# cartographer-project/cartographer

Measured on AMD Instinct MI355X. Metric: candidate poses scored/sec, higher is better.
Workload: dtype u8/int32; 1 GPU; C2: 2D FastCorrelativeScanMatcher MatchFullSubmap (branch and bound): 1000-point scan vs 1 400x400 submap(s) per GPU, depth 7, full-angle search, m...; submaps_per_gpu=1, rotations=2373, found=1

## Files before the change

### cartographer_amd/csrc/cmx_common.h

```cpp
#ifndef CMX_COMMON_H_
#define CMX_COMMON_H_

#include <hip/hip_runtime.h>

#include <cstdarg>
#include <cstdint>
#include <cstdio>
#include <cstring>
#include <functional>
#include <mutex>
#include <string>
#include <vector>

#include "../../include/cartographer_mi355x.h"

namespace cmx {

void SetLastError(const char* fmt, ...);
const char* LastError();

struct HipError {
  cmx_status status;
};

// ... 1 lines not shown
  do {                                                                             \
    hipError_t cmx_err__ = (expr);                                                 \
    if (cmx_err__ != hipSuccess) {                                                 \
      ::cmx::SetLastError("%s failed: %s (%s:%d)", #expr,                          \
                          hipGetErrorString(cmx_err__), __FILE__, __LINE__);       \
      throw ::cmx::HipError{cmx_err__ == hipErrorOutOfMemory ? CMX_OUT_OF_MEMORY   \
                                                             : CMX_DEVICE_ERROR};  \
    }                                                                              \
  } while (0)

#define CMX_REQUIRE(cond, ...)                       \
  do {                                               \
    if (!(cond)) {                                   \
      ::cmx::SetLastError(__VA_ARGS__);              \
      throw ::cmx::HipError{CMX_INVALID_ARGUMENT};   \
    }                                                \
  } while (0)

template <typename F>
cmx_status Guard(F&& body) {
  try {
    body();
    return CMX_OK;
  } catch (const HipError& e) {
    return e.status;
  } catch (const std::bad_alloc&) {
    SetLastError("host allocation failed");
    return CMX_OUT_OF_MEMORY;
  } catch (const std::exception& e) {
    SetLastError("exception: %s", e.what());
    return CMX_DEVICE_ERROR;
  }
}

#define CMX_DEBUG_OPTIONS(X)                                                                      \
  X(rt2d_legacy)                 \
  X(rt2d_tile)                                        \
  X(rt2d_groups)                                   \
  X(rt2d_target)                                    \
  X(rt2d_lds_kb)                                         \
  X(rt2d_no_image_cache)             \
  X(rt2d_parts)                                 \
  X(rt2d_host_par)         \
  X(rt2d_tables_serial)    \
  X(rt2d_first_part)       \
  X(rt2d_image_kernels)    \
  X(rt2d_no_lane)          \
  X(rt2d_parts_pool)       \
  X(rt2d_grid_share)       \
  X(rt2d_unfused)            \
  X(rt2d_no_bounds)        \
  X(rt2d_bounds)           \
  X(rt2d_bounds_fused)     \
  X(rt2d_bounds_level)     \
  X(rt2d_bounds_verify)    \
  X(rt2d_tsdf_batch_legacy)  \
  X(rt2d_tsdf_batch_bulk)  \
  X(rt2d_tsdf_verify)      \
  X(timeline)                  \
  X(trace)                       \
  X(host_trace)                          \
  X(launch_serial)         \
  X(sync)                      \
  X(no_copy_kernels)             \
  X(timing)                \
  X(no_direct_results)     \
  X(frontier_capacity)     \
  X(comm_virtual_ranks)    \
  X(comm_force_rccl)       \
  X(fast2d_unfused)                    \
  X(fast2d_store_scans)                   \
  X(fast2d_fused_threads)                            \
  X(fast2d_fanout)         \
  X(fast2d_group)          \
  X(fast2d_group_verify)   \
  X(fast2d_levels_per_stage)                                    \
  X(fast2d_wave_levels)                        \
  X(fast2d_xcd_affinity)                          \
  X(fast2d_dive)           \
  X(fast2d_queue)          \
  X(fast2d_queue_blocks)                \
  X(fast2d_queue_capacity)              \
  X(fast2d_queue_lost)       \
  X(filters_generic)       \
  X(fast3d_byte_loads)                             \
  X(fast3d_affinity)                              \
  X(fast3d_no_families)                             \
  X(fast3d_no_oct)                                         \
  X(fast3d_batch)                                                 \
  X(fast3d_chunk_cells)    \
  X(rt3d_legacy)                  \
  X(rt3d_no_tiles)                      \
  X(rt3d_verify)                  \
  X(rt3d_no_rotblocks)              \
  X(rt3d_rotblock_permille)  \
  X(rt3d_crosscheck)           \
  X(rt3d_expand_all)       \
  X(rt3d_unstaged)                                     \
  X(rt3d_no_boxes)                            \
  X(rt3d_report)                                             \
  X(rt3d_segments)                         \
  X(rt3d_group_rotations)                                  \
  X(rt3d_group_tile_kb)                                   \
  X(rt3d_group_float)                          \
  X(rt3d_cand_threads)                                   \
  X(rt3d_cand_rotations)                                    \
  X(rt3d_cand_tile_kb)
struct DebugOptions {
#define CMX_DEBUG_FIELD(name) int name = 0;
  CMX_DEBUG_OPTIONS(CMX_DEBUG_FIELD)
#undef CMX_DEBUG_FIELD
};
const DebugOptions& Debug();
bool DebugSet(const char* name, int value);

void UseDevice(int device);

void ParallelFor(int n, int serial_below, const std::function<void(int)>& fn);

class LaunchTurn {
 public:
  LaunchTurn();
  ~LaunchTurn();
  LaunchTurn(const LaunchTurn&) = delete;
  LaunchTurn& operator=(const LaunchTurn&) = delete;
 private:
  bool held_;
};

class HostLane {
 public:
  HostLane();
  ~HostLane();
  HostLane(const HostLane&) = delete;
  HostLane& operator=(const HostLane&) = delete;
  void Run(std::function<void()> fn);
  void Wait();
  bool own() const { return own_; }

 private:
  bool own_ = false, pending_ = false;
};

class DeviceBuffer {
 public:
  DeviceBuffer() = default;
  DeviceBuffer(const DeviceBuffer&) = delete;
  DeviceBuffer& operator=(const DeviceBuffer&) = delete;
  ~DeviceBuffer() { Free(); }
  void* Reserve(size_t bytes) {
    if (bytes > capacity_) {
      Free();
      const size_t want = bytes + bytes / 4 + 256;
      CMX_HIP(hipMalloc(&ptr_, want));
      capacity_ = want;
    }
    return ptr_;
  }
  template <typename T>
  T* ReserveAs(size_t count) { return static_cast<T*>(Reserve(count * sizeof(T))); }
  void* get() const { return ptr_; }
  size_t capacity() const { return capacity_; }
  void Free() {
    if (ptr_) (void)hipFree(ptr_);
    ptr_ = nullptr;
    capacity_ = 0;
// ... 127 lines not shown
```

### cartographer_amd/csrc/fast_2d.hip

```cpp
#include <algorithm>
#include <chrono>
#include <cstring>
#include <memory>
#include <type_traits>
#include <utility>

#include "fast_2d_device.h"
#include "fast_2d_internal.h"

namespace cmx {
namespace {

constexpr int kSeedsPerProblem = 64;

constexpr int kMaxStages = kMaxDepth + 2;

constexpr int kCountStride = 32;
constexpr int kQueues = 2048;
struct alignas(8) QueueCtl {
  int head;
  int reserved;
  int pad[30];
};
struct Counters {
// ... 869 lines not shown
                              __HIP_MEMORY_SCOPE_AGENT)) {
      const unsigned long long key =
          (static_cast<unsigned long long>(static_cast<unsigned>(nd.coarse_index)) << 32) | nd.path;
      atomicMin(&sel[p].key, key);
    }
  }
  __threadfence();
  __syncthreads();
  for (int i = threadIdx.x; i < total; i += blockDim.x) {
    Node2D nd;
    if (!leaf_at(i, &nd)) continue;
    const int p = NodeProblem(nd);
    const unsigned long long key =
        (static_cast<unsigned long long>(static_cast<unsigned>(nd.coarse_index)) << 32) | nd.path;
    if (__float_as_uint(nd.score) == states[p].best_bits &&
        __float_as_uint(nd.coarse_score) ==
            __hip_atomic_load(&sel[p].best_coarse_bits, __ATOMIC_RELAXED,
                              __HIP_MEMORY_SCOPE_AGENT) &&
        key == __hip_atomic_load(&sel[p].key, __ATOMIC_RELAXED, __HIP_MEMORY_SCOPE_AGENT)) {
      BestLeaf b;
      b.score = nd.score; b.scan = nd.scan; b.dx = nd.dx; b.dy = nd.dy;
      b.found = 1;
      b.ties = 1;
      b.pad0 = b.pad1 = 0;
      best[p] = b;
    }
  }
  __threadfence();
  __syncthreads();
  for (int i = threadIdx.x; i < total; i += blockDim.x) {
    Node2D nd;
    if (!leaf_at(i, &nd)) continue;
    const int p = NodeProblem(nd);
    if (__float_as_uint(nd.score) != states[p].best_bits) continue;
    const int scan = __hip_atomic_load(&best[p].scan, __ATOMIC_RELAXED, __HIP_MEMORY_SCOPE_AGENT);
    const int dx = __hip_atomic_load(&best[p].dx, __ATOMIC_RELAXED, __HIP_MEMORY_SCOPE_AGENT);
    const int dy = __hip_atomic_load(&best[p].dy, __ATOMIC_RELAXED, __HIP_MEMORY_SCOPE_AGENT);
    if (nd.scan != scan || nd.dx != dx || nd.dy != dy) atomicAdd(&best[p].ties, 1);
  }
}

__global__ void __launch_bounds__(1024)
SelectBestKernel(NodeList leaves, const ProblemState* __restrict__ states,
                 SelectState* __restrict__ sel, BestLeaf* __restrict__ best, int num_problems,
                 ProblemState* __restrict__ states_out, const Counters* __restrict__ counters,
                 CountersSummary* __restrict__ summary, const unsigned* __restrict__ tail_dev,
                 unsigned* __restrict__ tail_host, int tail_words) {
  SelectBestBody<false>(leaves, states, sel, best, num_problems, states_out, counters, summary);
  if (tail_host == nullptr) return;
  __threadfence();
  __syncthreads();
  for (int i = threadIdx.x; i < tail_words; i += blockDim.x)
    tail_host[i] = __hip_atomic_load(&tail_dev[i], __ATOMIC_RELAXED, __HIP_MEMORY_SCOPE_AGENT);
}

struct TreeQueue {
  unsigned long long* slots;
  int capacity;
  unsigned epoch;
};

__device__ __forceinline__ unsigned long long* QueueSlot(const TreeQueue& Q, int q, int slot) {
  return Q.slots + (static_cast<size_t>(q) * Q.capacity + slot) * 8;
}

__device__ __forceinline__ void StoreGranule(unsigned long long* g, unsigned epoch, unsigned value) {
  __hip_atomic_store(g, (static_cast<unsigned long long>(epoch) << 32) | value, __ATOMIC_RELAXED,
                     __HIP_MEMORY_SCOPE_AGENT);
}

__device__ __forceinline__ void StoreNodeGranules(const TreeQueue& Q, int q, int slot,
                                                  const Node2D& nd) {
  unsigned long long* g = QueueSlot(Q, q, slot);
  StoreGranule(g + 0, Q.epoch, static_cast<unsigned>(nd.problem));
  StoreGranule(g + 1, Q.epoch, static_cast<unsigned>(nd.scan));
  StoreGranule(g + 2, Q.epoch, static_cast<unsigned>(nd.dx));
  StoreGranule(g + 3, Q.epoch, static_cast<unsigned>(nd.dy));
  StoreGranule(g + 4, Q.epoch, __float_as_uint(nd.score));
  StoreGranule(g + 5, Q.epoch, static_cast<unsigned>(nd.coarse_index));
  StoreGranule(g + 6, Q.epoch, nd.path);
  StoreGranule(g + 7, Q.epoch, __float_as_uint(nd.coarse_score));
}

__device__ __forceinline__ void QueuePush(const TreeQueue& Q, Counters* __restrict__ counters,
                                          int q, bool keep, const Node2D& nd) {
  const int lane = threadIdx.x & 63;
  const unsigned long long mask = __ballot(keep);
  if (mask == 0) return;
  const int m = __popcll(mask);
  int first = 0;
  if (lane == 0)
    first = __hip_atomic_fetch_add(&counters->queue[q].reserved, m, __ATOMIC_RELAXED,
                                   __HIP_MEMORY_SCOPE_AGENT);
  first = __builtin_amdgcn_readfirstlane(first);
  if (first + m > Q.capacity && lane == 0)
    __hip_atomic_store(&counters->frontier_overflow, 1, __ATOMIC_RELAXED, __HIP_MEMORY_SCOPE_AGENT);
  if (keep) {
    const int slot = first + __popcll(mask & ((1ull << lane) - 1));
    if (slot < Q.capacity) StoreNodeGranules(Q, q, slot, nd);
  }
}

__device__ __forceinline__ void ReadSlot(const TreeQueue& Q, int q, int slot, Node2D* out,
                                         unsigned* slot_rereads) {
  const int lane = threadIdx.x & 63;
  const unsigned long long* g = QueueSlot(Q, q, slot);
  unsigned word = 0;
  for (;;) {
    bool ok = true;
    if (lane < 8) {
      const unsigned long long x = LoadAgent(&g[lane]);
      word = static_cast<unsigned>(x);
      ok = static_cast<unsigned>(x >> 32) == Q.epoch;
    }
    if (__all(ok)) break;
    ++*slot_rereads;
    __builtin_amdgcn_s_sleep(2);
  }
  out->problem = static_cast<int>(__builtin_amdgcn_readlane(word, 0));
  out->scan = static_cast<int>(__builtin_amdgcn_readlane(word, 1));
  out->dx = static_cast<int>(__builtin_amdgcn_readlane(word, 2));
  out->dy = static_cast<int>(__builtin_amdgcn_readlane(word, 3));
  out->score = __uint_as_float(__builtin_amdgcn_readlane(word, 4));
  out->coarse_index = static_cast<int>(__builtin_amdgcn_readlane(word, 5));
  out->path = __builtin_amdgcn_readlane(word, 6);
  out->coarse_score = __uint_as_float(__builtin_amdgcn_readlane(word, 7));
}

__device__ __forceinline__ bool TakeSlot(Counters* __restrict__ counters, int q, int slot) {
  int got = 0;
  if ((threadIdx.x & 63) == 0) {
    int expected = slot;
    got = __hip_atomic_compare_exchange_strong(&counters->queue[q].head, &expected, slot + 1,
                                               __ATOMIC_RELAXED, __ATOMIC_RELAXED,
                                               __HIP_MEMORY_SCOPE_AGENT) ? 1 : 0;
  }
  return __builtin_amdgcn_readfirstlane(got) != 0;
}

__device__ __forceinline__ bool PopHome(const TreeQueue& Q, Counters* __restrict__ counters,
                                        int home, Node2D* out, unsigned* lost_races,
                                        unsigned* slot_rereads) {
  for (;;) {
    const unsigned long long hr =
        LoadAgent(reinterpret_cast<const unsigned long long*>(&counters->queue[home].head));
    const int head = static_cast<int>(hr & 0xffffffffu);
    const int reserved = min(static_cast<int>(hr >> 32), Q.capacity);
    if (reserved <= head) return false;
    if (TakeSlot(counters, home, head)) {
      ReadSlot(Q, home, head, out, slot_rereads);
      return true;
    }
    ++*lost_races;
  }
}

__device__ __forceinline__ bool Steal(const TreeQueue& Q, Counters* __restrict__ counters,
                                      int home, int queues, unsigned salt, int windows,
                                      int max_lost, Node2D* out, unsigned* lost_races,
                                      unsigned* slot_rereads) {
  const int lane = threadIdx.x & 63;
  int lost = 0;
  for (int w = 0; w < windows; ++w) {
    const int base = static_cast<int>((static_cast<unsigned>(home) * 2654435761u + salt * 40503u + w * 64u) %
                                      static_cast<unsigned>(queues));
    const int mine = (base + lane) % queues;
    const unsigned long long hr =
        LoadAgent(reinterpret_cast<const unsigned long long*>(&counters->queue[mine].head));
    const int head = static_cast<int>(hr & 0xffffffffu);
    const int reserved = min(static_cast<int>(hr >> 32), Q.capacity);
    const unsigned long long avail = __ballot(reserved > head);
    if (avail == 0) continue;
    int skip = static_cast<int>((salt + home) % static_cast<unsigned>(__popcll(avail)));
    unsigned long long rest = avail;
    while (skip-- > 0) rest &= rest - 1;
    const int l = __ffsll(static_cast<long long>(rest)) - 1;
    const int q = (base + l) % queues;
    const int slot = __builtin_amdgcn_readlane(head, l);
    if (TakeSlot(counters, q, slot)) {
      ReadSlot(Q, q, slot, out, slot_rereads);
      return true;
    }
    ++*lost_races;
    if (++lost >= max_lost) return false;
    --w;
    ++salt;
  }
  return false;
}

constexpr int kChainCells = 16;
constexpr uint32_t kNoCell = 0x80008000u;

template <bool kRecompute>
__device__ __forceinline__ void LoadChainCells(const Fast2DProblem& P, int n, int scan,
                                               uint32_t (&cell)[kChainCells]) {
  const int lane = threadIdx.x & 63;
  const auto* pts = AsGlobal(P.discrete) + static_cast<size_t>(scan) * n;
  if constexpr (kRecompute) {
    const float2 rot = P.scan_rot[scan];
#pragma unroll
    for (int u = 0; u < kChainCells; ++u) cell[u] = kNoCell;
#pragma unroll 1
    for (int j = 0; j * kWave < n; ++j) {
      const int i = j * kWave + lane;
      const uint32_t c = i < n ? ScanCell(P, rot, i) : kNoCell;
#pragma unroll
      for (int u = 0; u < kChainCells; ++u) cell[u] = u == j ? c : cell[u];
    }
  } else {
#pragma unroll
    for (int j = 0; j < kChainCells; ++j) {
      const int i = j * kWave + lane;
      cell[j] = kNoCell;
      if (j * kWave < n) cell[j] = i < n ? pts[i] : kNoCell;
    }
  }
}

struct ChainLevel {
  int qx, qy, qtx;
  int half;
  int ax, ay;
  __amdgpu_buffer_rsrc_t quad_rsrc;
};

__device__ __forceinline__ ChainLevel MakeChainLevel(const Fast2DProblem& P, int child_level,
                                                     int dx, int dy) {
  const LevelDesc& Lm = P.level[child_level];
  ChainLevel L;
  L.half = 1 << child_level;
  L.ax = dx + 2 * L.half - 1;
  L.ay = dy + 2 * L.half - 1;
  L.qx = __builtin_amdgcn_readfirstlane(Lm.qx);
  L.qy = __builtin_amdgcn_readfirstlane(Lm.qy);
  L.qtx = __builtin_amdgcn_readfirstlane(Lm.qtx);
  const unsigned long long quads_address = reinterpret_cast<unsigned long long>(Lm.quads);
  const unsigned long long quads_uniform =
      static_cast<unsigned long long>(static_cast<unsigned>(
          __builtin_amdgcn_readfirstlane(static_cast<unsigned>(quads_address)))) |
      (static_cast<unsigned long long>(static_cast<unsigned>(
           __builtin_amdgcn_readfirstlane(static_cast<unsigned>(quads_address >> 32)))) << 32);
  const unsigned long long quad_bytes =
      static_cast<unsigned long long>((L.qy + 3) >> 2) * static_cast<unsigned>(L.qtx) * 128ull;
  L.quad_rsrc = __builtin_amdgcn_make_buffer_rsrc(
      reinterpret_cast<uint32_t*>(quads_uniform), 0, static_cast<int>(quad_bytes), 0x00020000);
  return L;
}

template <int kFirst, int kCount, bool kWantMax>
__device__ __forceinline__ void ChainGather(const ChainLevel& L, const uint32_t (&cell)[kChainCells],
                                            uint32_t* even, uint32_t* odd, int* seen_max) {
  typedef unsigned short Halves __attribute__((ext_vector_type(2)));
  uint32_t v[kCount];
#pragma unroll
  for (int u = 0; u < kCount; ++u) {
    const uint32_t p = cell[kFirst + u];
    const unsigned X = static_cast<unsigned>(static_cast<short>(p & 0xffffu) + L.ax);
    const unsigned Y = static_cast<unsigned>(static_cast<short>(p >> 16) + L.ay);
    const bool inside = X < static_cast<unsigned>(L.qx) && Y < static_cast<unsigned>(L.qy);
    const unsigned tile = __umul24(Y >> 2, static_cast<unsigned>(L.qtx)) + (X >> 3);
    const unsigned byte = (tile << 7) | ((Y & 3u) << 5) | ((X & 7u) << 2);
    v[u] = __builtin_amdgcn_raw_buffer_load_b32(L.quad_rsrc, inside ? byte : 0xfffffff0u, 0, 0);
  }
#pragma unroll
  for (int u = 0; u < kCount; ++u) {
    const uint32_t e = v[u] & 0x00ff00ffu, o = (v[u] >> 8) & 0x00ff00ffu;
    *even += e;
    *odd += o;
    if constexpr (kWantMax) {
      Halves eh, oh;
      __builtin_memcpy(&eh, &e, 4);
      __builtin_memcpy(&oh, &o, 4);
      const Halves m = __builtin_elementwise_max(eh, oh);
      *seen_max += static_cast<int>(max(m.x, m.y));
    }
  }
}

__global__ void __launch_bounds__(256)
DiveWaveKernel(const Fast2DProblem* __restrict__ problems, ProblemState* __restrict__ states, int n,
               NodeList leaves, Counters* __restrict__ counters) {
  const int problem = blockIdx.y;
  const Fast2DProblem& P = problems[problem];
  ProblemState& st = states[problem];
  if (st.error) return;
  __shared__ SeedScratch seed_scratch;
  const bool grouped = P.group > 1;
  const int seeds = grouped ? 1 : 4;
  const int want0 = static_cast<int>(blockIdx.x) * seeds;
  if (want0 >= kSeedsPerProblem) return;
  PickSeeds(P, n, want0, seeds, &seed_scratch);
  if (blockIdx.x == 0 && threadIdx.x == 0) st.coarse_total = seed_scratch.total;
  const int lane = threadIdx.x & 63;
  const int wave = __builtin_amdgcn_readfirstlane(threadIdx.x >> 6);
  if (grouped && wave >= kFusedGroup) return;
  int seed_scan = __builtin_amdgcn_readfirstlane(seed_scratch.found_scan[grouped ? 0 : wave]);
  if (seed_scan < 0) return;
  if (grouped) {
    seed_scan = seed_scan - seed_scan % kFusedGroup + wave;
    if (seed_scan >= P.num_scans) return;
  }
  const Node2D seed = CoarseNode(P, problem, seed_scan, P.scan_best[seed_scan].y);
  uint32_t cell[kChainCells];
  const bool stored =
      !P.recompute_scans ||
      (P.store_scans && !(ToScore(P, P.scan_best[seed_scan].x, n) < fmaxf(P.min_score, 0.f)));
  if (__builtin_amdgcn_readfirstlane(stored ? 1 : 0)) LoadChainCells<false>(P, n, seed_scan, cell);
  else LoadChainCells<true>(P, n, seed_scan, cell);
  const int4 bd = P.bounds[seed_scan];
  const int depth = P.depth;
  int dx = __builtin_amdgcn_readfirstlane(seed.dx), dy = __builtin_amdgcn_readfirstlane(seed.dy);
  float score = seed.score;
  unsigned long long scored = 0;
  for (int child_level = depth - 2; child_level >= 0; --child_level) {
    const ChainLevel L = MakeChainLevel(P, child_level, dx, dy);
    const bool vx = dx + L.half <= bd.y, vy = dy + L.half <= bd.w;
    uint32_t even = 0, odd = 0;
    if (n > 8 * kWave) ChainGather<0, 16, false>(L, cell, &even, &odd, nullptr);
    else if (n > 4 * kWave) ChainGather<0, 8, false>(L, cell, &even, &odd, nullptr);
    else ChainGather<0, 4, false>(L, cell, &even, &odd, nullptr);
    const int total[4] = {WaveSum(static_cast<int>(even & 0xffffu)), WaveSum(static_cast<int>(odd & 0xffffu)),
                          WaveSum(static_cast<int>(even >> 16)), WaveSum(static_cast<int>(odd >> 16))};
    int kbest = 0, nvalid = 0;
    float best_score = -1.f;
#pragma unroll
    for (int k = 0; k < 4; ++k) {
      const bool valid = ((k >> 1) == 0 || vx) && ((k & 1) == 0 || vy);
      const float sc = valid ? ToScore(P, total[k], n) : -1.f;
      nvalid += valid ? 1 : 0;
      if (sc >= 0.f && (k == 0 || sc > best_score)) { kbest = k; best_score = sc; }
    }
    kbest = __builtin_amdgcn_readfirstlane(kbest);
    dx += (kbest >> 1) * L.half;
    dy += (kbest & 1) * L.half;
    score = best_score;
    scored += nvalid;
  }
  if (lane == 0) {
    if (score > P.min_score) {
      Node2D leaf = seed;
      leaf.problem = problem;
      leaf.dx = dx;
      leaf.dy = dy;
      leaf.score = score;
      RecordLeaf(leaf, leaves, counters);
      atomicMax(&st.best_bits, __float_as_uint(score));
    }
    const int shard = (blockIdx.x * 4 + wave) & (kStatShards - 1);
    atomicAdd(&st.scored_shard[shard], scored);
    atomicAdd(&st.expanded_shard[shard], static_cast<unsigned long long>(depth - 1));
  }
}

__device__ __forceinline__ void RecordLeafAgent(const Node2D& leaf, const NodeList& leaves,
                                                int sub, Counters* __restrict__ counters) {
  const int slot = ListReserve(leaves, sub, 1);
  if (slot >= leaves.sub_capacity) {
    __hip_atomic_store(&counters->leaf_overflow, 1, __ATOMIC_RELAXED, __HIP_MEMORY_SCOPE_AGENT);
    return;
  }
  unsigned long long v[4];
  __builtin_memcpy(v, &leaf, sizeof(Node2D));
  unsigned long long* at = reinterpret_cast<unsigned long long*>(
      &leaves.nodes[static_cast<size_t>(sub) * leaves.sub_capacity + slot]);
#pragma unroll
  for (int k = 0; k < 4; ++k)
    __hip_atomic_store(&at[k], v[k], __ATOMIC_RELAXED, __HIP_MEMORY_SCOPE_AGENT);
}

__global__ void __launch_bounds__(256)
TreeQueueKernel(const Fast2DProblem* __restrict__ problems, ProblemState* __restrict__ states, int n,
                NodeList in, TreeQueue Q, NodeList leaves, Counters* __restrict__ counters,
                SelectState* __restrict__ sel, BestLeaf* __restrict__ best_out, int num_problems,
                ProblemState* __restrict__ states_out, CountersSummary* __restrict__ summary,
                const unsigned* __restrict__ tail_dev, unsigned* __restrict__ tail_host,
                int tail_words, int counters_trace, int max_lost) {
  static_assert(sizeof(Node2D) == 32, "a node is eight words: eight granules, four leaf stores");
  const int lane = threadIdx.x & 63;
  const int wave_id = blockIdx.x * 4 + __builtin_amdgcn_readfirstlane(threadIdx.x >> 6);
  const int num_waves = gridDim.x * 4;
  const int queues = min(num_waves, kQueues);
  const int home = wave_id % queues;
  unsigned steals = 0;
  unsigned long long scored = 0, expanded = 0;
  unsigned gathers = 0;
  unsigned q_pops = 0, q_lost = 0, q_rereads = 0, q_pushed = 0, q_listed = 0, q_chains = 0;
  int stat_problem = -1;
  const auto flush_stats = [&]() {
    if (lane == 0 && stat_problem >= 0 && expanded) {
      ProblemState& st = states[stat_problem];
      atomicAdd(&st.scored_shard[wave_id & (kStatShards - 1)], scored);
      atomicAdd(&st.expanded_shard[wave_id & (kStatShards - 1)], expanded);
    }
    scored = expanded = 0;
  };
  const int in_slots = ListMaxCount(in) * kSubLists;
  int round = 0;
  Node2D mine{};
  unsigned mine_bits = 0;
  bool round_loaded = false, share_done = false;
  bool pushed_any = false;
  Node2D nd;
  for (;;) {
    bool have = false;
    while (!have && !share_done) {
      if (!round_loaded) {
        if (wave_id + static_cast<long long>(round) * 64 * num_waves >= in_slots) { share_done = true; break; }
        const long long i = wave_id + (static_cast<long long>(round) * 64 + lane) * num_waves;
        ++round;
        mine_bits = 0;
        if (i < in_slots) {
          const int in_sub = static_cast<int>(i & (kSubLists - 1)), j = static_cast<int>(i / kSubLists);
          if (j < min(in.counts[in_sub * kCountStride], in.sub_capacity)) {
            mine = in.nodes[static_cast<size_t>(in_sub) * in.sub_capacity + j];
            mine_bits = max(__float_as_uint(fmaxf(mine.score, 0.f)), 1u);
          }
        }
        round_loaded = true;
      }
      const unsigned top = static_cast<unsigned>(WaveMax(static_cast<int>(mine_bits)));
      const float bound_now = __uint_as_float(LoadAgent(&states[0].best_bits));
      if (top == 0 || (num_problems == 1 && __uint_as_float(top) < bound_now)) {
        round_loaded = false;
        continue;
      }
      const int l = __ffsll(static_cast<long long>(__ballot(mine_bits == top))) - 1;
      nd.problem = __builtin_amdgcn_readlane(mine.problem, l);
      nd.scan = __builtin_amdgcn_readlane(mine.scan, l);
      nd.dx = __builtin_amdgcn_readlane(mine.dx, l);
      nd.dy = __builtin_amdgcn_readlane(mine.dy, l);
      nd.score = __uint_as_float(__builtin_amdgcn_readlane(__float_as_uint(mine.score), l));
      nd.coarse_index = __builtin_amdgcn_readlane(mine.coarse_index, l);
      nd.path = __builtin_amdgcn_readlane(mine.path, l);
      nd.coarse_score =
          __uint_as_float(__builtin_amdgcn_readlane(__float_as_uint(mine.coarse_score), l));
      if (lane == l) mine_bits = 0;
      have = true;
      ++q_listed;
    }
    if (!have) {
      if (!(pushed_any && PopHome(Q, counters, home, &nd, &q_lost, &q_rereads)) &&
          !Steal(Q, counters, home, queues, ++steals, 2, max_lost, &nd, &q_lost, &q_rereads))
        break;
      ++q_pops;
    }
    const int problem = __builtin_amdgcn_readfirstlane(NodeProblem(nd));
    const Fast2DProblem& P = problems[problem];
    ProblemState& st = states[problem];
    float best = __uint_as_float(LoadAgent(&st.best_bits));
    if (nd.score < best) continue;
    if (problem != stat_problem) { flush_stats(); stat_problem = problem; }
    ++q_chains;
    uint32_t cell[kChainCells];
    LoadChainCells<false>(P, n, nd.scan, cell);
    const int4 bd = P.bounds[nd.scan];
    const float min_score = P.min_score;
    for (;;) {
      const int child_level = __builtin_amdgcn_readfirstlane(NodeLevel(nd) - 1);
      const int ndx = __builtin_amdgcn_readfirstlane(nd.dx), ndy = __builtin_amdgcn_readfirstlane(nd.dy);
      const ChainLevel L = MakeChainLevel(P, child_level, ndx, ndy);
      const int half = L.half;
      const bool vx = ndx + half <= bd.y, vy = ndy + half <= bd.w;
      const int parent_ub = SumUpperBound(P, nd.score, n);
      uint32_t even = 0, odd = 0;
      int seen_max = 0;
      bool dead = false;
      const auto gather = [&](auto first_tag, auto count_tag) {
        ChainGather<decltype(first_tag)::value, decltype(count_tag)::value, true>(L, cell, &even,
                                                                                  &odd, &seen_max);
      };
      gather(std::integral_constant<int, 0>{}, std::integral_constant<int, 4>{});
      gathers += 4;
      if (n > 4 * kWave) {
        const int most = static_cast<int>(max(max(even & 0xffffu, even >> 16),
                                              max(odd & 0xffffu, odd >> 16)));
        if (ToScore(P, parent_ub - WaveSum(seen_max - most), n) < best) {
          dead = true;
        } else {
          if (n > 8 * kWave) {
            gather(std::integral_constant<int, 4>{}, std::integral_constant<int, 12>{});
            gathers += 12;
          } else {
            gather(std::integral_constant<int, 4>{}, std::integral_constant<int, 4>{});
            gathers += 4;
          }
        }
      }
      ++expanded;
      scored += (1 + (vx ? 1 : 0)) * (1 + (vy ? 1 : 0));
      if (dead) break;
      const int total[4] = {WaveSum(static_cast<int>(even & 0xffffu)), WaveSum(static_cast<int>(odd & 0xffffu)),
                            WaveSum(static_cast<int>(even >> 16)), WaveSum(static_cast<int>(odd >> 16))};
      float sc[4];
#pragma unroll
      for (int k = 0; k < 4; ++k) {
        const bool valid = ((k >> 1) == 0 || vx) && ((k & 1) == 0 || vy);
        sc[k] = valid ? ToScore(P, total[k], n) : -1.f;
      }
      const int k = lane & 3;
      const float mine = k == 0 ? sc[0] : (k == 1 ? sc[1] : (k == 2 ? sc[2] : sc[3]));
      int rank = 0;
#pragma unroll
      for (int o = 0; o < 4; ++o)
        if (o != k && sc[o] >= 0.f && (sc[o] > mine || (sc[o] == mine && o < k))) ++rank;
      best = fmaxf(best, __uint_as_float(LoadAgent(&st.best_bits)));
      const bool keep = lane < 4 && mine >= 0.f && mine >= best;
      const int kbest = __ffsll(static_cast<long long>(__ballot(lane < 4 && mine >= 0.f && rank == 0))) - 1;
      Node2D child;
      child.problem = problem | (child_level << 24);
      child.scan = nd.scan;
      child.dx = nd.dx + (k >> 1) * half;
      child.dy = nd.dy + (k & 1) * half;
      child.score = mine;
      child.coarse_index = nd.coarse_index;
      child.path = nd.path | (static_cast<unsigned>(rank) << (2 * child_level));
      child.coarse_score = nd.coarse_score;
      const bool best_kept = (__ballot(keep) >> kbest) & 1ull;
      if (child_level == 0) {
        if (best_kept && lane == kbest && child.score > min_score) {
          RecordLeafAgent(child, leaves, wave_id & (kSubLists - 1), counters);
          atomicMax(&st.best_bits, __float_as_uint(child.score));
        }
        break;
      }
      if (!best_kept) break;
      const bool others = keep && lane != kbest;
      if (__ballot(others)) {
        QueuePush(Q, counters, home, others, child);
        pushed_any = true;
        q_pushed += __popcll(__ballot(others));
      }
      nd.problem = child.problem;
      nd.dx = __builtin_amdgcn_readlane(child.dx, kbest);
      nd.dy = __builtin_amdgcn_readlane(child.dy, kbest);
      nd.score = __uint_as_float(__builtin_amdgcn_readlane(__float_as_uint(child.score), kbest));
      nd.path = __builtin_amdgcn_readlane(child.path, kbest);
    }
  }
  __shared__ unsigned long long s_scored[4], s_expanded[4];
  __shared__ unsigned s_gathers[4];
  __shared__ unsigned s_queue_stats[8];
  __shared__ int s_problem[4];
  if (threadIdx.x < 8) s_queue_stats[threadIdx.x] = 0;
  __syncthreads();
  if (lane == 0 && counters_trace) {
    atomicAdd(&s_queue_stats[0], q_pops);
    atomicAdd(&s_queue_stats[1], q_lost);
    atomicAdd(&s_queue_stats[2], q_rereads);
    atomicAdd(&s_queue_stats[3], q_pushed);
    atomicAdd(&s_queue_stats[4], q_listed);
    atomicAdd(&s_queue_stats[5], q_chains);
  }
  __shared__ int s_last;
  if (lane == 0) {
    const int w = threadIdx.x >> 6;
    s_scored[w] = scored;
    s_expanded[w] = expanded;
    s_gathers[w] = gathers;
    s_problem[w] = expanded ? stat_problem : -1;
  }
  asm volatile("s_waitcnt vmcnt(0)" ::: "memory");
  __syncthreads();
  if (threadIdx.x == 0) {
    unsigned g = 0;
    for (int w = 0; w < 4; ++w) {
      g += s_gathers[w];
      if (s_problem[w] < 0) continue;
      unsigned long long sc = s_scored[w], ex = s_expanded[w];
      for (int v = w + 1; v < 4; ++v)
        if (s_problem[v] == s_problem[w]) { sc += s_scored[v]; ex += s_expanded[v]; s_problem[v] = -1; }
      ProblemState& st = states[s_problem[w]];
      atomicAdd(&st.scored_shard[blockIdx.x & (kStatShards - 1)], sc);
      atomicAdd(&st.expanded_shard[blockIdx.x & (kStatShards - 1)], ex);
    }
    if (g) atomicAdd(&counters->gathers_shard[(blockIdx.x & 15) * kCountStride], g);
    if (counters_trace)
      for (int k = 0; k < 6; ++k)
        if (s_queue_stats[k])
          atomicAdd(&counters->queue_stats[(blockIdx.x & 15) * kCountStride + k], s_queue_stats[k]);
    asm volatile("s_waitcnt vmcnt(0)" ::: "memory");
    s_last = __hip_atomic_fetch_add(&counters->blocks_done, 1, __ATOMIC_RELAXED,
                                    __HIP_MEMORY_SCOPE_AGENT) == static_cast<int>(gridDim.x) - 1;
  }
  __syncthreads();
  if (!s_last) return;
  SelectBestBody<true>(leaves, states, sel, best_out, num_problems, states_out, counters, summary);
  if (tail_host == nullptr) return;
  __threadfence();
  __syncthreads();
  for (int i = threadIdx.x; i < tail_words; i += blockDim.x)
    tail_host[i] = __hip_atomic_load(&tail_dev[i], __ATOMIC_RELAXED, __HIP_MEMORY_SCOPE_AGENT);
}

__global__ void __launch_bounds__(1024)
SelectDepthOneKernel(const Fast2DProblem* __restrict__ problems,
                     const ProblemState* __restrict__ states, int n, BestLeaf* __restrict__ best,
                     ProblemState* __restrict__ states_out) {
  const int problem = blockIdx.x;
  const Fast2DProblem& P = problems[problem];
  __shared__ unsigned long long keys[16];
  __shared__ int s_total;
  if (threadIdx.x == 0) s_total = 0;
  __syncthreads();
  unsigned long long key = 0;
  int total = 0;
  for (int s = threadIdx.x; s < P.num_scans; s += blockDim.x) {
    total += P.coarse_dims[s].x * P.coarse_dims[s].y;
    const int2 b = P.scan_best[s];
    const unsigned long long k = (static_cast<unsigned long long>(static_cast<unsigned>(b.x)) << 32) |
                                 static_cast<unsigned>(0x7fffffff - s);
    key = k > key ? k : key;
  }
  key = WaveMaxU64(key);
  total = WaveSum(total);
  if ((threadIdx.x & 63) == 0) {
    keys[threadIdx.x >> 6] = key;
    if (total) atomicAdd(&s_total, total);
  }
  __syncthreads();
  if (threadIdx.x == 0) {
    ProblemState st = states[problem];
    st.coarse_total = s_total;
    states_out[problem] = st;
    for (int w = 1; w < 16; ++w) key = keys[w] > key ? keys[w] : key;
    BestLeaf b{};
    if (!states[problem].error && P.num_scans > 0) {
      const int s = 0x7fffffff - static_cast<int>(key & 0xffffffffu);
      const int2 sb = P.scan_best[s];
      const float score = ToScore(P, sb.x, n);
      if (score > P.min_score) {
        const int2 dims = P.coarse_dims[s];
        const int4 bd = P.bounds[s];
        b.found = 1; b.score = score; b.scan = s;
        b.dx = bd.x + sb.y / dims.y;
        b.dy = bd.z + sb.y % dims.y;
// ... 64 lines not shown
  frontier_sub = frontier_capacity / kSubLists;
  const int leaf_capacity = capacity(0, 1 << 20);
  Node2D* d_leaves = ws.dev[12].ReserveAs<Node2D>(leaf_capacity);
  d_counters = reinterpret_cast<Counters*>(batch.d_misc);
  d_tail = SearchTail(batch.d_misc + sizeof(Counters), num);
  leaf_list = NodeList{d_leaves, d_counters->leaves, leaf_capacity / kSubLists};
  h_tail = SearchTail(static_cast<char*>(ws.pinned[3].Reserve(SearchTail::Bytes(num))), num);
  direct = Debug().no_direct_results == 0 && h_tail.bytes % sizeof(unsigned) == 0;
}

void SearchRun::FetchResults(bool published) {
  if (!published)
    SmallCopyAsync(h_tail.base, d_tail.base, h_tail.bytes, false, ws.stream);
  const auto t0 = std::chrono::steady_clock::now();
  CMX_HIP(hipStreamSynchronize(ws.stream));
  g_host_wait_ns += std::chrono::duration_cast<std::chrono::nanoseconds>(
                        std::chrono::steady_clock::now() - t0).count();
}

void SearchRun::PrepareStrictRetry() {
  CMX_REQUIRE(num_chunks < (1 << 12), "branch-and-bound overflow not resolvable");
  if (h_tail.summary->frontier_overflow) num_chunks *= 4;
  strict = 1;
  for (int p = 0; p < num; ++p) {
    const float floor_score = std::max(batch.h_problems[p].min_score, 0.f);
    unsigned floor_bits;
    std::memcpy(&floor_bits, &floor_score, sizeof(float));
    if (h_tail.states[p].best_bits > floor_bits) h_tail.states[p].best_bits -= 1;
  }
  CMX_HIP(hipMemcpyAsync(batch.d_states, h_tail.states, num * sizeof(ProblemState),
                         hipMemcpyHostToDevice, ws.stream));
  CMX_HIP(hipMemsetAsync(d_counters, 0, sizeof(Counters), ws.stream));
}

void RunDepthOne(SearchRun& run) {
  Workspace& ws = run.ws;
  SelectDepthOneKernel<<<run.num, 1024, 0, ws.stream>>>(
      run.batch.d_problems, run.batch.d_states, run.n, run.d_tail.best, run.d_tail.states);
  CMX_HIP(hipGetLastError());
  RecordEvent(ws.ev_end, ws.stream);
  run.FetchResults(false);
}

bool ChainWalkPossible(const SearchRun& run) {
  bool chain_ok = run.n <= kChainCells * kWave;
  for (const Fast2DProblem& P : run.batch.h_problems)
    for (int l = 0; l + 1 < run.depth; ++l)
      chain_ok = chain_ok && static_cast<unsigned long long>((P.level[l].qy + 3) >> 2) *
                                     static_cast<unsigned>(P.level[l].qtx) * 128ull < (1ull << 31);
  return chain_ok;
}

bool QueueSearchPossible(const SearchRun& run) {
  bool queue_ok = QueueSearchWanted(run.n, run.num) && ChainWalkPossible(run);
  for (const Fast2DProblem& P : run.batch.h_problems)
    queue_ok = queue_ok && (P.recompute_scans == 0 || P.store_scans != 0);
  return queue_ok;
}

enum class QueueOutcome { kDone, kLeafOverflow, kQueueOverflow };

QueueOutcome RunQueueSearch(SearchRun& run, std::unique_ptr<LaunchTurn> turn) {
  Workspace& ws = run.ws;
  const PreparedBatch& batch = run.batch;
  BatchResult* result = run.result;
  const int num = run.num, n = run.n;
  const long long wanted = std::max<long long>(1ll << 20, 65536ll * num);
  int sub_capacity = static_cast<int>(std::min<long long>(wanted, 1ll << 23) / kQueues);
  if (Debug().fast2d_queue_capacity > 0) sub_capacity = Debug().fast2d_queue_capacity;
  TreeQueue queue;
  queue.capacity = sub_capacity;
  queue.slots = static_cast<unsigned long long*>(ws.tagged[0].Acquire(
      static_cast<size_t>(kQueues) * sub_capacity * 8 * sizeof(unsigned long long), ws.stream,
      &queue.epoch));
  run.d_front[0] = ws.dev[10].ReserveAs<Node2D>(run.frontier_capacity);
  FilterCoarseKernel<<<dim3(DivUp(batch.max_scans, 4), num), 256, 0, ws.stream>>>(
      batch.d_problems, batch.d_states, n, 0, 1, 0, 0, run.Front(0),
      run.d_counters);
  run.Mark("filter");
  RecordEvent(ws.ev_x0, ws.stream);
  const int blocks = Debug().fast2d_queue_blocks > 0
                         ? Debug().fast2d_queue_blocks
                         : std::min(2048, 256 * std::max(1, (num + 3) / 4));
  TreeQueueKernel<<<blocks, 256, 0, ws.stream>>>(
      batch.d_problems, batch.d_states, n, run.Front(0), queue, run.leaf_list, run.d_counters,
      run.d_tail.sel, run.d_tail.best, num, run.d_tail.states, run.d_tail.summary,
      run.d_tail.words(), run.PublishTo(), run.h_tail.num_words(),
      batch.trace && batch.trace->enabled() ? 1 : 0,
      Debug().fast2d_queue_lost > 0 ? Debug().fast2d_queue_lost : 3);
  run.Mark("queue");
  CMX_HIP(hipGetLastError());
  RecordEvent(ws.ev_x1, ws.stream);
  result->expansion_launches = 1;
  RecordEvent(ws.ev_end, ws.stream);
  turn.reset();
  run.FetchResults(run.direct);
  const CountersSummary& h_counters = *run.h_tail.summary;
  result->expansion_lookups = 64ll * h_counters.wave_gathers;
  for (int p = 0; p < num; ++p)
    for (int k = 0; k < kStatShards; ++k)
      result->expansion_nodes += run.h_tail.states[p].expanded_shard[k];
  if (h_counters.leaf_overflow) return QueueOutcome::kLeafOverflow;
  if (h_counters.frontier_overflow) return QueueOutcome::kQueueOverflow;
  return QueueOutcome::kDone;
}

void RunLevelSynchronous(SearchRun& run) {
  Workspace& ws = run.ws;
  const PreparedBatch& batch = run.batch;
  BatchResult* result = run.result;
  const int num = run.num, n = run.n;
  const CountersSummary& h_counters = *run.h_tail.summary;
  const int kLevelsPerStage = std::max(0, Debug().fast2d_levels_per_stage);
  const int kWaveLevels = Debug().fast2d_wave_levels > 0 ? Debug().fast2d_wave_levels - 1 : -1;
  const int levels_per_stage = kLevelsPerStage > 0 ? kLevelsPerStage : (num < 4 ? kMaxDepth : 2);
  const int wave_levels = kWaveLevels >= 0 ? kWaveLevels : (num < 4 ? 1 : 2);
  const int affinity_override = Debug().fast2d_xcd_affinity;
  const int affinity = affinity_override ? affinity_override - 1 : (num >= 16 ? 1 : 0);
  const int wide_blocks = std::min(4096, 1024 * std::max(1, (num + 3) / 4));
  const int narrow_blocks = std::min(4096, 512 * std::max(1, (num + 3) / 4));
  run.d_front[0] = ws.dev[10].ReserveAs<Node2D>(run.frontier_capacity);
  run.d_front[1] = ws.dev[11].ReserveAs<Node2D>(run.frontier_capacity);
  for (;;) {
    const int strict = run.strict;
    for (int chunk = 0; chunk < run.num_chunks; ++chunk) {
      if (chunk > 0 || strict)
        CMX_HIP(hipMemsetAsync(run.d_counters->frontier, 0, sizeof(run.d_counters->frontier),
                               ws.stream));
      FilterCoarseKernel<<<dim3(DivUp(batch.max_scans, 4), num), 256, 0, ws.stream>>>(
          batch.d_problems, batch.d_states, n, chunk, run.num_chunks, strict, affinity,
          run.Front(0), run.d_counters);
      run.Mark("filter");
      int stage = 0;
      int top = run.depth - 1;
      const bool timed = !strict && chunk == 0 && num >= 4;
      if (timed) RecordEvent(ws.ev_x0, ws.stream);
      for (int used = 0; used < wave_levels && top - 1 >= 1; ++used, --top, ++stage) {
        ExpandWaveKernel<<<used == 0 ? wide_blocks : narrow_blocks, 256, 0, ws.stream>>>(
            batch.d_problems, batch.d_states, n, run.Front(stage), strict, affinity,
            run.Front(stage + 1), run.d_counters);
        run.Mark("wave");
      }
      if (timed) {
        RecordEvent(ws.ev_x1, ws.stream);
        result->expansion_launches = stage;
      }
      for (; top > 0; top -= levels_per_stage, ++stage) {
        const int stop = std::max(0, top - levels_per_stage);
        SubtreeKernel<<<narrow_blocks, 256, 0, ws.stream>>>(
            batch.d_problems, batch.d_states, n, run.Front(stage), stop, strict,
            run.Front(stage + 1), run.leaf_list, run.d_counters);
        run.Mark("subtree");
      }
    }
    SelectBestKernel<<<1, 1024, 0, ws.stream>>>(
        run.leaf_list, batch.d_states, run.d_tail.sel, run.d_tail.best, num, run.d_tail.states,
        run.d_counters, run.d_tail.summary, run.d_tail.words(), run.PublishTo(),
        run.h_tail.num_words());
    run.Mark("select");
    CMX_HIP(hipGetLastError());
    RecordEvent(ws.ev_end, ws.stream);
    run.FetchResults(run.direct);
    if (!strict) {
      for (int st = 0; st < result->expansion_launches; ++st)
        result->expansion_nodes += h_counters.frontier_total[st];
      result->expansion_lookups = 64ll * h_counters.wave_gathers;
    }
// ... 84 lines not shown
```

Measured before the change: 10.79 billion candidates/s.

## Overlap chain gathers with deferred queue pushes and speculative loads in tree kernel

Templates the tree-queue kernel on a chain mode. The default mode 0 issues all gather loads for a level up front, before the early-kill test. It also splits queue pushes into an atomic reservation issued before the gathers and slot writes completed after them. Node, bounds and cell loads are hoisted ahead of the bound check, and the per-wave queue statistics are packed into lanes to save scalar registers. This hides memory latency of atomics and gathers, at the cost of wasted loads on pruned nodes and extra register pressure.

```diff
diff --git a/cartographer_amd/csrc/cmx_common.h b/cartographer_amd/csrc/cmx_common.h
--- a/cartographer_amd/csrc/cmx_common.h
+++ b/cartographer_amd/csrc/cmx_common.h
@@ -107,6 +107,7 @@
   X(fast2d_queue_blocks)                \
   X(fast2d_queue_capacity)              \
   X(fast2d_queue_lost)       \
+  X(fast2d_chain)          \
   X(filters_generic)       \
   X(fast3d_byte_loads)                             \
   X(fast3d_affinity)                              \
diff --git a/cartographer_amd/csrc/fast_2d.hip b/cartographer_amd/csrc/fast_2d.hip
--- a/cartographer_amd/csrc/fast_2d.hip
+++ b/cartographer_amd/csrc/fast_2d.hip
@@ -975,23 +975,38 @@
   StoreGranule(g + 7, Q.epoch, __float_as_uint(nd.coarse_score));
 }
 
+__device__ __forceinline__ int QueueReserve(Counters* __restrict__ counters, int q,
+                                            unsigned long long mask) {
+  auto* reserved = AsGlobal(&counters->queue[q].reserved);
+  asm("" : "+v"(reserved));
+  int first = 0;
+  if ((threadIdx.x & 63) == 0 && mask != 0)
+    first = __hip_atomic_fetch_add(reserved, __popcll(mask), __ATOMIC_RELAXED,
+                                   __HIP_MEMORY_SCOPE_AGENT);
+  return first;
+}
+
+__device__ __forceinline__ void QueueComplete(const TreeQueue& Q, Counters* __restrict__ counters,
+                                              int q, unsigned long long mask, int ticket,
+                                              const Node2D& nd) {
+  const int lane = threadIdx.x & 63;
+  const int m = __popcll(mask);
+  const int first = __builtin_amdgcn_readfirstlane(ticket);
+  if (first + m > Q.capacity && lane == 0)
+    __hip_atomic_store(&counters->frontier_overflow, 1, __ATOMIC_RELAXED, __HIP_MEMORY_SCOPE_AGENT);
+  if ((mask >> lane) & 1ull) {
+    const int slot = first + static_cast<int>(__builtin_amdgcn_mbcnt_hi(
+                                 static_cast<unsigned>(mask >> 32),
+                                 __builtin_amdgcn_mbcnt_lo(static_cast<unsigned>(mask), 0u)));
+    if (slot < Q.capacity) StoreNodeGranules(Q, q, slot, nd);
+  }
+}
+
 __device__ __forceinline__ void QueuePush(const TreeQueue& Q, Counters* __restrict__ counters,
                                           int q, bool keep, const Node2D& nd) {
-  const int lane = threadIdx.x & 63;
   const unsigned long long mask = __ballot(keep);
   if (mask == 0) return;
-  const int m = __popcll(mask);
-  int first = 0;
-  if (lane == 0)
-    first = __hip_atomic_fetch_add(&counters->queue[q].reserved, m, __ATOMIC_RELAXED,
-                                   __HIP_MEMORY_SCOPE_AGENT);
-  first = __builtin_amdgcn_readfirstlane(first);
-  if (first + m > Q.capacity && lane == 0)
-    __hip_atomic_store(&counters->frontier_overflow, 1, __ATOMIC_RELAXED, __HIP_MEMORY_SCOPE_AGENT);
-  if (keep) {
-    const int slot = first + __popcll(mask & ((1ull << lane) - 1));
-    if (slot < Q.capacity) StoreNodeGranules(Q, q, slot, nd);
-  }
+  QueueComplete(Q, counters, q, mask, QueueReserve(counters, q, mask), nd);
 }
 
 __device__ __forceinline__ void ReadSlot(const TreeQueue& Q, int q, int slot, Node2D* out,
@@ -1018,6 +1033,19 @@
   out->coarse_index = static_cast<int>(__builtin_amdgcn_readlane(word, 5));
   out->path = __builtin_amdgcn_readlane(word, 6);
   out->coarse_score = __uint_as_float(__builtin_amdgcn_readlane(word, 7));
+}
+
+__device__ __forceinline__ Node2D UniformNode(const Node2D& nd) {
+  Node2D u;
+  u.problem = __builtin_amdgcn_readfirstlane(nd.problem);
+  u.scan = __builtin_amdgcn_readfirstlane(nd.scan);
+  u.dx = __builtin_amdgcn_readfirstlane(nd.dx);
+  u.dy = __builtin_amdgcn_readfirstlane(nd.dy);
+  u.score = __uint_as_float(__builtin_amdgcn_readfirstlane(__float_as_uint(nd.score)));
+  u.coarse_index = __builtin_amdgcn_readfirstlane(nd.coarse_index);
+  u.path = __builtin_amdgcn_readfirstlane(nd.path);
+  u.coarse_score = __uint_as_float(__builtin_amdgcn_readfirstlane(__float_as_uint(nd.coarse_score)));
+  return u;
 }
 
 __device__ __forceinline__ bool TakeSlot(Counters* __restrict__ counters, int q, int slot) {
@@ -1141,11 +1169,9 @@
   return L;
 }
 
-template <int kFirst, int kCount, bool kWantMax>
-__device__ __forceinline__ void ChainGather(const ChainLevel& L, const uint32_t (&cell)[kChainCells],
-                                            uint32_t* even, uint32_t* odd, int* seen_max) {
-  typedef unsigned short Halves __attribute__((ext_vector_type(2)));
-  uint32_t v[kCount];
+template <int kFirst, int kCount>
+__device__ __forceinline__ void ChainIssue(const ChainLevel& L, const uint32_t (&cell)[kChainCells],
+                                           uint32_t* v) {
 #pragma unroll
   for (int u = 0; u < kCount; ++u) {
     const uint32_t p = cell[kFirst + u];
@@ -1156,6 +1182,12 @@
     const unsigned byte = (tile << 7) | ((Y & 3u) << 5) | ((X & 7u) << 2);
     v[u] = __builtin_amdgcn_raw_buffer_load_b32(L.quad_rsrc, inside ? byte : 0xfffffff0u, 0, 0);
   }
+}
+
+template <int kCount, bool kWantMax>
+__device__ __forceinline__ void ChainSum(const uint32_t* v, uint32_t* even, uint32_t* odd,
+                                         int* seen_max) {
+  typedef unsigned short Halves __attribute__((ext_vector_type(2)));
 #pragma unroll
   for (int u = 0; u < kCount; ++u) {
     const uint32_t e = v[u] & 0x00ff00ffu, o = (v[u] >> 8) & 0x00ff00ffu;
@@ -1169,6 +1201,14 @@
       *seen_max += static_cast<int>(max(m.x, m.y));
     }
   }
+}
+
+template <int kFirst, int kCount, bool kWantMax>
+__device__ __forceinline__ void ChainGather(const ChainLevel& L, const uint32_t (&cell)[kChainCells],
+                                            uint32_t* even, uint32_t* odd, int* seen_max) {
+  uint32_t v[kCount];
+  ChainIssue<kFirst, kCount>(L, cell, v);
+  ChainSum<kCount, kWantMax>(v, even, odd, seen_max);
 }
 
 __global__ void __launch_bounds__(256)
@@ -1262,6 +1302,7 @@
     __hip_atomic_store(&at[k], v[k], __ATOMIC_RELAXED, __HIP_MEMORY_SCOPE_AGENT);
 }
 
+template <int kChain>
 __global__ void __launch_bounds__(256)
 TreeQueueKernel(const Fast2DProblem* __restrict__ problems, ProblemState* __restrict__ states, int n,
                 NodeList in, TreeQueue Q, NodeList leaves, Counters* __restrict__ counters,
@@ -1276,15 +1317,17 @@
   const int queues = min(num_waves, kQueues);
   const int home = wave_id % queues;
   unsigned steals = 0;
-  unsigned long long scored = 0, expanded = 0;
+  unsigned scored = 0, expanded = 0;
   unsigned gathers = 0;
-  unsigned q_pops = 0, q_lost = 0, q_rereads = 0, q_pushed = 0, q_listed = 0, q_chains = 0;
+  enum { kPops, kLost, kRereads, kPushed, kListed, kChains, kQueueStats };
+  unsigned q_stats = 0;
+  const auto count = [&](int which, unsigned by) { q_stats += lane == which ? by : 0u; };
   int stat_problem = -1;
   const auto flush_stats = [&]() {
     if (lane == 0 && stat_problem >= 0 && expanded) {
       ProblemState& st = states[stat_problem];
-      atomicAdd(&st.scored_shard[wave_id & (kStatShards - 1)], scored);
-      atomicAdd(&st.expanded_shard[wave_id & (kStatShards - 1)], expanded);
+      atomicAdd(&st.scored_shard[wave_id & (kStatShards - 1)], static_cast<unsigned long long>(scored));
+      atomicAdd(&st.expanded_shard[wave_id & (kStatShards - 1)], static_cast<unsigned long long>(expanded));
     }
     scored = expanded = 0;
   };
@@ -1298,22 +1341,34 @@
   for (;;) {
     bool have = false;
     while (!have && !share_done) {
+      unsigned round_bound_bits = 0;
       if (!round_loaded) {
         if (wave_id + static_cast<long long>(round) * 64 * num_waves >= in_slots) { share_done = true; break; }
+        if constexpr (kChain != 1) round_bound_bits = LoadAgent(&states[0].best_bits);
         const long long i = wave_id + (static_cast<long long>(round) * 64 + lane) * num_waves;
         ++round;
         mine_bits = 0;
         if (i < in_slots) {
           const int in_sub = static_cast<int>(i & (kSubLists - 1)), j = static_cast<int>(i / kSubLists);
-          if (j < min(in.counts[in_sub * kCountStride], in.sub_capacity)) {
+          if constexpr (kChain == 1) {
+            if (j < min(in.counts[in_sub * kCountStride], in.sub_capacity)) {
+              mine = in.nodes[static_cast<size_t>(in_sub) * in.sub_capacity + j];
+              mine_bits = max(__float_as_uint(fmaxf(mine.score, 0.f)), 1u);
+            }
+          } else {
+            const int count = in.counts[in_sub * kCountStride];
             mine = in.nodes[static_cast<size_t>(in_sub) * in.sub_capacity + j];
-            mine_bits = max(__float_as_uint(fmaxf(mine.score, 0.f)), 1u);
+            if (j < min(count, in.sub_capacity))
+              mine_bits = max(__float_as_uint(fmaxf(mine.score, 0.f)), 1u);
           }
         }
         round_loaded = true;
+      } else if constexpr (kChain != 1) {
+        round_bound_bits = LoadAgent(&states[0].best_bits);
       }
       const unsigned top = static_cast<unsigned>(WaveMax(static_cast<int>(mine_bits)));
-      const float bound_now = __uint_as_float(LoadAgent(&states[0].best_bits));
+      if constexpr (kChain == 1) round_bound_bits = LoadAgent(&states[0].best_bits);
+      const float bound_now = __uint_as_float(round_bound_bits);
       if (top == 0 || (num_problems == 1 && __uint_as_float(top) < bound_now)) {
         round_loaded = false;
         continue;
@@ -1330,25 +1385,43 @@
           __uint_as_float(__builtin_amdgcn_readlane(__float_as_uint(mine.coarse_score), l));
       if (lane == l) mine_bits = 0;
       have = true;
-      ++q_listed;
+      count(kListed, 1);
     }
     if (!have) {
-      if (!(pushed_any && PopHome(Q, counters, home, &nd, &q_lost, &q_rereads)) &&
-          !Steal(Q, counters, home, queues, ++steals, 2, max_lost, &nd, &q_lost, &q_rereads))
-        break;
-      ++q_pops;
-    }
+      unsigned lost = 0, rereads = 0;
+      const bool got = (pushed_any && PopHome(Q, counters, home, &nd, &lost, &rereads)) ||
+                       Steal(Q, counters, home, queues, ++steals, 2, max_lost, &nd, &lost, &rereads);
+      count(kLost, lost);
+      count(kRereads, rereads);
+      if (!got) break;
+      count(kPops, 1);
+    }
+    if constexpr (kChain != 1) nd = UniformNode(nd);
     const int problem = __builtin_amdgcn_readfirstlane(NodeProblem(nd));
     const Fast2DProblem& P = problems[problem];
     ProblemState& st = states[problem];
     float best = __uint_as_float(LoadAgent(&st.best_bits));
+    uint32_t cell[kChainCells];
+    int4 bd;
+    if constexpr (kChain != 1) {
+      const auto* bounds = AsGlobal(reinterpret_cast<const int*>(P.bounds + nd.scan));
+      bd = make_int4(bounds[0], bounds[1], bounds[2], bounds[3]);
+      LoadChainCells<false>(P, n, nd.scan, cell);
+    }
     if (nd.score < best) continue;
     if (problem != stat_problem) { flush_stats(); stat_problem = problem; }
-    ++q_chains;
-    uint32_t cell[kChainCells];
-    LoadChainCells<false>(P, n, nd.scan, cell);
-    const int4 bd = P.bounds[nd.scan];
+    count(kChains, 1);
+    if constexpr (kChain == 1) {
+      LoadChainCells<false>(P, n, nd.scan, cell);
+      bd = P.bounds[nd.scan];
+    }
     const float min_score = P.min_score;
+    unsigned pending = 0;
+    unsigned pending_score[4] = {0, 0, 0, 0};
+    unsigned pending_ranks = 0;
+    int pending_dx = 0, pending_dy = 0;
+    unsigned pending_path = 0;
+    if constexpr (kChain != 1) __builtin_amdgcn_s_waitcnt(0x0f70);
     for (;;) {
       const int child_level = __builtin_amdgcn_readfirstlane(NodeLevel(nd) - 1);
       const int ndx = __builtin_amdgcn_readfirstlane(nd.dx), ndy = __builtin_amdgcn_readfirstlane(nd.dy);
@@ -1363,21 +1436,77 @@
         ChainGather<decltype(first_tag)::value, decltype(count_tag)::value, true>(L, cell, &even,
                                                                                   &odd, &seen_max);
       };
-      gather(std::integral_constant<int, 0>{}, std::integral_constant<int, 4>{});
-      gathers += 4;
-      if (n > 4 * kWave) {
-        const int most = static_cast<int>(max(max(even & 0xffffu, even >> 16),
-                                              max(odd & 0xffffu, odd >> 16)));
-        if (ToScore(P, parent_ub - WaveSum(seen_max - most), n) < best) {
-          dead = true;
-        } else {
-          if (n > 8 * kWave) {
-            gather(std::integral_constant<int, 4>{}, std::integral_constant<int, 12>{});
-            gathers += 12;
+      int pending_ticket = 0;
+      if constexpr (kChain != 1) pending_ticket = QueueReserve(counters, home, pending);
+      if constexpr (kChain != 1) {
+        const auto expand = [&](auto rest_tag) {
+          constexpr int kRest = decltype(rest_tag)::value;
+          const unsigned bound_bits = LoadAgent(&st.best_bits);
+          uint32_t v[4 + (kRest ? kRest : 1)];
+          ChainIssue<0, 4>(L, cell, v);
+          if constexpr (kRest > 0 && kChain == 0) {
+            ChainIssue<4, kRest>(L, cell, v + 4);
+            asm volatile("" ::: "memory");
+          }
+          gathers += kChain == 0 ? 4 + kRest : 4;
+          best = fmaxf(best, __uint_as_float(bound_bits));
+          ChainSum<4, true>(v, &even, &odd, &seen_max);
+          if constexpr (kRest > 0) {
+            const int most = static_cast<int>(max(max(even & 0xffffu, even >> 16),
+                                                  max(odd & 0xffffu, odd >> 16)));
+            if (__builtin_amdgcn_readfirstlane(
+                    ToScore(P, parent_ub - WaveSum(seen_max - most), n) < best ? 1 : 0)) {
+              dead = true;
+            } else {
+              if constexpr (kChain == 2) {
+                ChainIssue<4, kRest>(L, cell, v + 4);
+                gathers += kRest;
+              }
+              ChainSum<kRest, true>(v + 4, &even, &odd, &seen_max);
+            }
+          }
+        };
+        if (n > 8 * kWave) expand(std::integral_constant<int, 12>{});
+        else if (n > 4 * kWave) expand(std::integral_constant<int, 4>{});
+        else expand(std::integral_constant<int, 0>{});
+      } else {
+        gather(std::integral_constant<int, 0>{}, std::integral_constant<int, 4>{});
+        gathers += 4;
+        if (n > 4 * kWave) {
+          const int most = static_cast<int>(max(max(even & 0xffffu, even >> 16),
+                                                max(odd & 0xffffu, odd >> 16)));
+          if (ToScore(P, parent_ub - WaveSum(seen_max - most), n) < best) {
+            dead = true;
           } else {
-            gather(std::integral_constant<int, 4>{}, std::integral_constant<int, 4>{});
-            gathers += 4;
+            if (n > 8 * kWave) {
+              gather(std::integral_constant<int, 4>{}, std::integral_constant<int, 12>{});
+              gathers += 12;
+            } else {
+              gather(std::integral_constant<int, 4>{}, std::integral_constant<int, 4>{});
+              gathers += 4;
+            }
           }
+        }
+      }
+      if constexpr (kChain != 1) {
+        __builtin_amdgcn_s_waitcnt(0x0f70);
+        if (pending) {
+          const int level = child_level + 1, k = lane & 3;
+          int scan = nd.scan, coarse_index = nd.coarse_index;
+          unsigned coarse_bits = __float_as_uint(nd.coarse_score);
+          asm volatile("" : "+s"(scan), "+s"(coarse_index), "+s"(coarse_bits));
+          Node2D child;
+          child.problem = problem | (level << 24);
+          child.scan = scan;
+          child.dx = pending_dx + ((k >> 1) << level);
+          child.dy = pending_dy + ((k & 1) << level);
+          child.score = __uint_as_float(k == 0 ? pending_score[0] : (k == 1 ? pending_score[1] :
+                                        (k == 2 ? pending_score[2] : pending_score[3])));
+          child.coarse_index = coarse_index;
+          child.path = pending_path | (((pending_ranks >> (2 * k)) & 3u) << (2 * level));
+          child.coarse_score = __uint_as_float(coarse_bits);
+          QueueComplete(Q, counters, home, pending, pending_ticket, child);
+          pending = 0;
         }
       }
       ++expanded;
@@ -1397,7 +1526,7 @@
 #pragma unroll
       for (int o = 0; o < 4; ++o)
         if (o != k && sc[o] >= 0.f && (sc[o] > mine || (sc[o] == mine && o < k))) ++rank;
-      best = fmaxf(best, __uint_as_float(LoadAgent(&st.best_bits)));
+      if constexpr (kChain == 1) best = fmaxf(best, __uint_as_float(LoadAgent(&st.best_bits)));
       const bool keep = lane < 4 && mine >= 0.f && mine >= best;
       const int kbest = __ffsll(static_cast<long long>(__ballot(lane < 4 && mine >= 0.f && rank == 0))) - 1;
       Node2D child;
@@ -1419,10 +1548,24 @@
       }
       if (!best_kept) break;
       const bool others = keep && lane != kbest;
-      if (__ballot(others)) {
-        QueuePush(Q, counters, home, others, child);
+      const unsigned push = __builtin_amdgcn_readfirstlane(static_cast<unsigned>(__ballot(others)));
+      if constexpr (kChain == 1) {
+        if (push) QueuePush(Q, counters, home, others, child);
+      } else {
+        pending = push;
+        pending_ranks = 0;
+#pragma unroll
+        for (int o = 0; o < 4; ++o) {
+          pending_score[o] = __builtin_amdgcn_readfirstlane(__float_as_uint(sc[o]));
+          pending_ranks |= static_cast<unsigned>(__builtin_amdgcn_readlane(rank, o)) << (2 * o);
+        }
+        pending_dx = ndx;
+        pending_dy = ndy;
+        pending_path = nd.path;
+      }
+      if (push) {
         pushed_any = true;
-        q_pushed += __popcll(__ballot(others));
+        count(kPushed, __popc(push));
       }
       nd.problem = child.problem;
       nd.dx = __builtin_amdgcn_readlane(child.dx, kbest);
@@ -1437,14 +1580,7 @@
   __shared__ int s_problem[4];
   if (threadIdx.x < 8) s_queue_stats[threadIdx.x] = 0;
   __syncthreads();
-  if (lane == 0 && counters_trace) {
-    atomicAdd(&s_queue_stats[0], q_pops);
-    atomicAdd(&s_queue_stats[1], q_lost);
-    atomicAdd(&s_queue_stats[2], q_rereads);
-    atomicAdd(&s_queue_stats[3], q_pushed);
-    atomicAdd(&s_queue_stats[4], q_listed);
-    atomicAdd(&s_queue_stats[5], q_chains);
-  }
+  if (lane < kQueueStats && counters_trace) atomicAdd(&s_queue_stats[lane], q_stats);
   __shared__ int s_last;
   if (lane == 0) {
     const int w = threadIdx.x >> 6;
@@ -1675,7 +1811,10 @@
   const int blocks = Debug().fast2d_queue_blocks > 0
                          ? Debug().fast2d_queue_blocks
                          : std::min(2048, 256 * std::max(1, (num + 3) / 4));
-  TreeQueueKernel<<<blocks, 256, 0, ws.stream>>>(
+  const int chain = Debug().fast2d_chain;
+  const auto tree_kernel = chain == 1 ? TreeQueueKernel<1> : (chain == 2 ? TreeQueueKernel<2>
+                                                                          : TreeQueueKernel<0>);
+  tree_kernel<<<blocks, 256, 0, ws.stream>>>(
       batch.d_problems, batch.d_states, n, run.Front(0), queue, run.leaf_list, run.d_counters,
       run.d_tail.sel, run.d_tail.best, num, run.d_tail.states, run.d_tail.summary,
       run.d_tail.words(), run.PublishTo(), run.h_tail.num_words(),
```

Measured after the change: 10.82 billion candidates/s (median of 3 runs). About the same (+0.3%).
